# ChainSafe/lumenos

Measured on AMD Instinct MI355X. Metric: prove_eval_seconds_16384x4096, lower is better.
Workload: dtype u64; 1 GPU; Encode+Commit+InnerProduct(r,b)+QueryCols 16384x4096 LogN=14 L=12 K=2 rhoInv=2 queries=309; parallelism=1 GPU: the whole job resident in HBM

## Files before the change

### lumenos_amd/csrc/lm_common.h

```cpp
#pragma once
#include <hip/hip_runtime.h>

#include <algorithm>
#include <cstdarg>
#include <cstdint>
#include <cstdio>
#include <map>
#include <memory>
#include <mutex>
#include <set>
#include <string>
#include <utility>
#include <vector>

#include "../../include/lumenos_hip.h"
#include "lm_arith.h"
#include "lm_dev.h"

#define LM_MAX_LIMBS LUMEN_MAX_LIMBS

struct lm_modmap {
    uint32_t period;
    uint8_t idx[LM_MAX_LIMBS];
};

struct lm_mods {
    mod_t m[LM_MAX_LIMBS];
};

struct lm_prof_entry {
    double total_ms = 0;
    uint64_t launches = 0;
    uint64_t units = 0;
};

struct lm_galois_key {
    lm_dev<u64> d_key;
    lm_dev<uint32_t> d_index;
    lm_dev<uint32_t> d_inv_index;
};

struct lumen_set {
    uint32_t count = 0;
    uint32_t nl = 0;
    uint32_t logw = 0;
    u64 *d = nullptr;
    size_t words = 0;
    bool owner = true;
    lumen_ctx *home = nullptr;
};

struct lm_shared {
    std::recursive_mutex mu;
    lm_dev<tw_t> tw_fwd;
    lm_dev<tw_t> tw_inv;
    std::vector<uint64_t> roots;
    uint32_t fieldN = 0;
    lm_dev<tw_t> scal;
    std::map<uint64_t, lm_galois_key> gkeys;
    std::map<std::string, std::shared_ptr<void>> ext;
};

struct lm_tuning {
    uint32_t ks_batch = 64;
    uint32_t ks_lanes = 0;
    int32_t ks_fused_digits = -1;
    uint32_t ks_close_fused = 1;
    uint32_t debug = 0;
    uint32_t modup_tgroup = 3, moddown_tgroup = 1;
    uint32_t ks_placement = 6;
    uint32_t batch_chunks = 0;
    uint32_t rccl_shared_device = 0;
};

struct lumen_ctx {
    lm_tuning tune;
    std::recursive_mutex mu;
    std::shared_ptr<lm_shared> sh;
    int device = 0;
    hipStream_t stream = nullptr;
    hipStream_t stream2 = nullptr;
    hipEvent_t ev_fork = nullptr, ev_join = nullptr;
    hipStream_t stream_aux = nullptr;
    hipEvent_t ev_aux = nullptr;
    hipEvent_t ev_xdep = nullptr;
    uint32_t aux_digests = 0;
    const u64 *aux_lo = nullptr, *aux_hi = nullptr;
    uint8_t *aux_host = nullptr;
    size_t aux_host_cap = 0;
    void *stage_host = nullptr;
    size_t stage_cap = 0;
    hipEvent_t ev_stage = nullptr;
    void *io_host[2] = {nullptr, nullptr};
    hipEvent_t ev_io[2] = {nullptr, nullptr};
    uint32_t logN = 0, N = 0, L = 0, K = 0;
    uint64_t T = 0;
    uint64_t mod[LM_MAX_LIMBS] = {0};
    uint64_t psi[LM_MAX_LIMBS] = {0};
    lm_mods mods;
    tw_t ninv[LM_MAX_LIMBS];
    std::vector<uint64_t> &roots;
    uint32_t &fieldN;
    std::map<uint64_t, lm_galois_key> &gkeys;
    std::map<std::string, std::shared_ptr<void>> &ext;
    uint64_t mul_counter = 0;
    std::map<std::string, lm_dev<unsigned char>> scratch;
    struct pool_block {
        void *p;
        hipEvent_t ready;
    };
    std::multimap<size_t, pool_block> pool;
    size_t pool_bytes = 0;
    std::set<const void *> lds_attr_done;
    bool prof = false;
    std::map<std::string, lm_prof_entry> prof_tab;
    struct pending_ev {
        std::string name;
        hipEvent_t a, b;
        uint64_t units;
    };
    std::vector<pending_ev> prof_pending;
    std::vector<hipEvent_t> ev_pool;
    hipEvent_t tm0 = nullptr, tm1 = nullptr;
    std::string err;
    explicit lumen_ctx(std::shared_ptr<lm_shared> s)
        : sh(std::move(s)), roots(sh->roots), fieldN(sh->fieldN), gkeys(sh->gkeys), ext(sh->ext) {}
};

static inline size_t lm_ctw(const lumen_ctx *ctx, const lumen_set *s);
#define LM_FULL_WIDTH(ctx, set, what) \
    LM_CHECK(ctx, (set)->logw == 0, "%s: lane-sharded set (1/%u of every limb) where a full-width set is required", what, 1u << (set)->logw)

#define LM_ENTER(ctx)                                             \
    std::lock_guard<std::recursive_mutex> lm_lock_((ctx)->mu);    \
    (void)hipSetDevice((ctx)->device);                            \
    (void)hipGetLastError()
#define LM_SHARED_LOCK(ctx) std::lock_guard<std::recursive_mutex> lm_shlock_((ctx)->sh->mu)

template <class T>
static inline std::shared_ptr<T> lm_ext_get(lumen_ctx *ctx, const std::string &key) {
    LM_SHARED_LOCK(ctx);
    auto it = ctx->ext.find(key);
    return it == ctx->ext.end() ? std::shared_ptr<T>() : std::static_pointer_cast<T>(it->second);
}
static inline void lm_ext_put(lumen_ctx *ctx, const std::string &key, std::shared_ptr<void> v) {
    LM_SHARED_LOCK(ctx);
    ctx->ext[key] = std::move(v);
}

static inline size_t lm_ctw(const lumen_ctx *ctx, const lumen_set *s) { return (size_t)2 * s->nl * (ctx->N >> s->logw); }

void lm_sync_all(lumen_ctx *ctx);
void *lm_stage(lumen_ctx *ctx, size_t bytes);
int lm_h2d_staged(lumen_ctx *ctx, void *dev, const void *host, size_t bytes);
bool lm_host_is_pinned(const void *p);
int lm_h2d(lumen_ctx *ctx, void *dev, const void *host, size_t bytes);
int lm_d2h(lumen_ctx *ctx, void *host, const void *dev, size_t bytes, bool wait);
int lm_h2d_rows(lumen_ctx *ctx, void *dev, size_t dpitch, const void *host, size_t spitch, size_t width, size_t height);

int lm_fail(lumen_ctx *ctx, const char *fmt, ...);
extern thread_local std::string lm_global_err;

#define LM_HIP(ctx, call)                                                                  \
    do {                                                                                   \
        hipError_t e_ = (call);                                                            \
        if (e_ != hipSuccess)                                                              \
            return lm_fail(ctx, "%s failed: %s (%s:%d)", #call, hipGetErrorString(e_),     \
                           __FILE__, __LINE__);                                            \
    } while (0)

#define LM_CHECK(ctx, cond, ...)                    \
    do {                                            \
        if (!(cond)) return lm_fail(ctx, __VA_ARGS__); \
    } while (0)

template <class... P, class... A>
static inline int lm_launch_flat(lumen_ctx *ctx, void (*kernel)(P...), size_t threads, A &&...args) {
    hipLaunchKernelGGL(kernel, dim3((uint32_t)((threads + 255) / 256)), dim3(256), 0, ctx->stream, std::forward<A>(args)...);
    LM_HIP(ctx, hipGetLastError());
    return 0;
}

struct lm_set_guard {
    lumen_ctx *ctx;
    lumen_set *s;
    lm_set_guard(lumen_ctx *c, lumen_set *x) : ctx(c), s(x) {}
    ~lm_set_guard() {
        if (s) lumen_set_destroy(ctx, s);
    }
    lumen_set *release() {
        lumen_set *r = s;
        s = nullptr;
        return r;
    }
    lm_set_guard(lm_set_guard &&o) : ctx(o.ctx), s(o.release()) {}
    lm_set_guard &operator=(const lm_set_guard &) = delete;
};

void lm_set_release_async(lumen_ctx *ctx, lumen_set *set);

void *lm_scratch(lumen_ctx *ctx, const char *name, size_t bytes);
void lm_scratch_adopt(lumen_ctx *ctx, const char *name, void *p, size_t bytes);

struct lm_prof_scope {
    lumen_ctx *ctx;
    const char *name;
    uint64_t units;
    hipEvent_t a = nullptr;
    lm_prof_scope(lumen_ctx *c, const char *n, uint64_t u);
    ~lm_prof_scope();
};
void lm_prof_resolve(lumen_ctx *ctx);

static inline uint64_t h_mulmod(uint64_t a, uint64_t b, uint64_t q) {
    return (uint64_t)(((u128)a * b) % q);
}
static inline uint64_t h_powmod(uint64_t a, uint64_t e, uint64_t q) {
    uint64_t r = 1 % q;
    a %= q;
    while (e) {
        if (e & 1) r = h_mulmod(r, a, q);
        a = h_mulmod(a, a, q);
        e >>= 1;
    }
    return r;
}
static inline uint64_t h_invmod(uint64_t a, uint64_t q) { return h_powmod(a, q - 2, q); }
static inline tw_t h_tw(uint64_t w, uint64_t q) {
    tw_t t;
    t.w = w;
    t.wp = (u64)((((u128)w) << 64) / q);
    return t;
}
static inline uint64_t h_r64_mod(uint64_t q) { return (uint64_t)((((u128)1) << 64) % q); }
static inline uint64_t h_p_mod(const lumen_ctx *ctx, uint64_t q) {
    uint64_t P = 1 % q;
    for (uint32_t a = 0; a < ctx->K; a++) P = h_mulmod(P, ctx->mod[ctx->L + a] % q, q);
    return P;
}
static inline uint32_t h_bitrev(uint32_t x, int bits) {
    uint32_t r = 0;
    for (int i = 0; i < bits; i++) r = (r << 1) | ((x >> i) & 1);
    return r;
}

int lm_launch_ntt(lumen_ctx *ctx, u64 *d, uint32_t npoly, const lm_modmap &map, bool inverse);
struct lm_ninv_t;
int lm_launch_ntt_strided(lumen_ctx *ctx, const u64 *src, size_t src_poly_stride, u64 *dst,
                          size_t dst_poly_stride, uint32_t npoly, const lm_modmap &map, bool inverse,
                          const char *prof_name, const lm_ninv_t *inv_scale = nullptr);
int lm_launch_ntt_subring(lumen_ctx *ctx, uint32_t logn, const tw_t *tw, tw_t ninv_scale, const u64 *src,
                          size_t src_poly_stride, u64 *dst, size_t dst_poly_stride, uint32_t npoly,
                          uint32_t mod_idx, bool inverse, const mod_t *explicit_mod = nullptr);
mod_t lm_make_mod(uint64_t q);
void lm_build_tw(uint64_t q, uint64_t psi, uint32_t logN, std::vector<tw_t> &fwd, std::vector<tw_t> &inv);
int lm_rescale_polys(lumen_ctx *ctx, const u64 *src, uint32_t nl, u64 *dst, uint32_t target,
                     uint32_t npoly, u64 *work, u64 *tbuf);
int lm_rescale_coef_ready(lumen_ctx *ctx);
int lm_rescale_polys_from_coef(lumen_ctx *ctx, const u64 *coef, uint32_t nl, u64 *dst, uint32_t target, uint32_t npoly);
lm_modmap lm_map_q(uint32_t nl);
lm_modmap lm_map_p(const lumen_ctx *ctx);
int lm_encode_dev(lumen_ctx *ctx, const lumen_set *matrix, const u64 *dzero, uint32_t rho_inv, lumen_set **encoded);
int lm_poly_eval_check(lumen_ctx *ctx, const uint64_t *values, uint32_t rows, uint32_t count, uint64_t first_column,
                       uint32_t cols, const char *what);
int lm_poly_eval_enqueue(lumen_ctx *ctx, const uint64_t *values, uint32_t rows, uint32_t count, uint64_t first_column,
                         uint32_t cols, uint64_t z, const char *what);
int lm_poly_eval_finish(lumen_ctx *ctx, uint64_t *partial);
hipEvent_t lm_ev_get(lumen_ctx *ctx);
```

### lumenos_amd/csrc/lm_ctx.hip

```cpp
#include <cstring>
#include <thread>

#include "lm_ntt_dev.h"

thread_local std::string lm_global_err;

int lm_fail(lumen_ctx *ctx, const char *fmt, ...) {
    char buf[1024];
    va_list ap;
    va_start(ap, fmt);
    vsnprintf(buf, sizeof(buf), fmt, ap);
    va_end(ap);
    if (ctx) ctx->err = buf;
    lm_global_err = buf;
    fprintf(stderr, "[lumenos_hip] error: %s\n", buf);
    return 1;
}

void *lm_scratch(lumen_ctx *ctx, const char *name, size_t bytes) {
    auto &e = ctx->scratch[name];
    if (e && e.count() >= bytes) return e.get();
    if (e) lm_sync_all(ctx);
    return e.alloc(ctx, bytes, name) ? nullptr : e.get();
}

void lm_scratch_adopt(lumen_ctx *ctx, const char *name, void *p, size_t bytes) {
    auto &e = ctx->scratch[name];
    if (e.get() == p) (void)e.release();
    if (e) lm_sync_all(ctx);
    e = lm_dev<unsigned char>((unsigned char *)p, bytes);
}

void lm_sync_all(lumen_ctx *ctx) {
    if (ctx->stream) hipStreamSynchronize(ctx->stream);
    if (ctx->stream2) hipStreamSynchronize(ctx->stream2);
    if (ctx->stream_aux) hipStreamSynchronize(ctx->stream_aux);
}

void *lm_stage(lumen_ctx *ctx, size_t bytes) {
    if (ctx->ev_stage) hipEventSynchronize(ctx->ev_stage);
    if (ctx->stage_cap < bytes) {
        if (ctx->stage_host) hipHostFree(ctx->stage_host);
        ctx->stage_host = nullptr, ctx->stage_cap = 0;
        if (hipHostMalloc(&ctx->stage_host, bytes, hipHostMallocDefault) != hipSuccess) {
            lm_fail(ctx, "hipHostMalloc(%zu) for host staging failed", bytes);
            return nullptr;
        }
        ctx->stage_cap = bytes;
    }
    return ctx->stage_host;
}

int lm_h2d_staged(lumen_ctx *ctx, void *dev, const void *host, size_t bytes) {
    void *h = lm_stage(ctx, bytes);
    if (!h) return 1;
    memcpy(h, host, bytes);
    LM_HIP(ctx, hipMemcpyAsync(dev, h, bytes, hipMemcpyHostToDevice, ctx->stream));
    LM_HIP(ctx, hipEventRecord(ctx->ev_stage, ctx->stream));
    return 0;
}

hipEvent_t lm_ev_get(lumen_ctx *ctx) {
    if (!ctx->ev_pool.empty()) {
        hipEvent_t e = ctx->ev_pool.back();
        ctx->ev_pool.pop_back();
        return e;
    }
    hipEvent_t e = nullptr;
    hipEventCreate(&e);
    return e;
}

lm_prof_scope::lm_prof_scope(lumen_ctx *c, const char *n, uint64_t u) : ctx(c), name(n), units(u) {
    if (!ctx->prof) return;
    a = lm_ev_get(ctx);
    hipEventRecord(a, ctx->stream);
}
lm_prof_scope::~lm_prof_scope() {
    if (!ctx->prof || !a) return;
    hipEvent_t b = lm_ev_get(ctx);
    hipEventRecord(b, ctx->stream);
    ctx->prof_pending.push_back({name, a, b, units});
}

void lm_prof_resolve(lumen_ctx *ctx) {
    if (ctx->prof_pending.empty()) return;
    for (auto &p : ctx->prof_pending) {
        float ms = 0;
        if (hipEventSynchronize(p.b) == hipSuccess && hipEventElapsedTime(&ms, p.a, p.b) == hipSuccess) {
            auto &e = ctx->prof_tab[p.name];
            e.total_ms += ms;
            e.launches += 1;
            e.units += p.units;
        } else {
            (void)hipGetLastError();
        }
        ctx->ev_pool.push_back(p.a);
        ctx->ev_pool.push_back(p.b);
    }
    ctx->prof_pending.clear();
}

lm_modmap lm_map_q(uint32_t nl) {
    lm_modmap m;
    m.period = nl;
    for (uint32_t i = 0; i < LM_MAX_LIMBS; i++) m.idx[i] = (uint8_t)(i < nl ? i : 0);
    return m;
}

lm_modmap lm_map_p(const lumen_ctx *ctx) {
    lm_modmap m;
    m.period = ctx->K;
    for (uint32_t i = 0; i < LM_MAX_LIMBS; i++) m.idx[i] = (uint8_t)(ctx->L + (i < ctx->K ? i : 0));
    return m;
}

mod_t lm_make_mod(uint64_t q) {
    mod_t m;
    m.q = q;
    m.qinv64 = (u64)((((u128)1) << 64) / q);
    u64 inv = 1;
    for (int it = 0; it < 6; it++) inv *= 2 - (u64)q * inv;
    m.qneg = (u64)0 - inv;
    u64 r = h_r64_mod(q);
    m.r2 = h_mulmod(r, r, q);
    return m;
}

void lm_build_tw(uint64_t q, uint64_t psi, uint32_t logN, std::vector<tw_t> &fwd, std::vector<tw_t> &inv) {
    uint32_t N = 1u << logN;
    fwd.resize(N);
    inv.resize(N);
    uint64_t psi_inv = h_invmod(psi, q), cf = 1, cb = 1;
    for (uint32_t j = 0; j < N; j++) {
        uint32_t r = h_bitrev(j, (int)logN);
        fwd[r] = h_tw(cf, q);
        inv[r] = h_tw(cb, q);
        cf = h_mulmod(cf, psi, q);
        cb = h_mulmod(cb, psi_inv, q);
    }
}

static void pool_drain(lumen_ctx *ctx) {
    for (auto &kv : ctx->pool) {
        hipFree(kv.second.p);
        if (kv.second.ready) ctx->ev_pool.push_back(kv.second.ready);
    }
    ctx->pool.clear();
    ctx->pool_bytes = 0;
}

static int ctx_private_init(lumen_ctx *ctx) {
    LM_HIP(ctx, hipSetDevice(ctx->device));
    LM_HIP(ctx, hipStreamCreate(&ctx->stream));
    LM_HIP(ctx, hipStreamCreate(&ctx->stream2));
    LM_HIP(ctx, hipEventCreateWithFlags(&ctx->ev_fork, hipEventDisableTiming));
    LM_HIP(ctx, hipEventCreateWithFlags(&ctx->ev_join, hipEventDisableTiming));
    LM_HIP(ctx, hipStreamCreate(&ctx->stream_aux));
    LM_HIP(ctx, hipEventCreateWithFlags(&ctx->ev_aux, hipEventDisableTiming));
    LM_HIP(ctx, hipEventCreateWithFlags(&ctx->ev_stage, hipEventDisableTiming));
    LM_HIP(ctx, hipEventCreateWithFlags(&ctx->ev_xdep, hipEventDisableTiming));
    LM_HIP(ctx, hipEventCreate(&ctx->tm0));
    LM_HIP(ctx, hipEventCreate(&ctx->tm1));
    return 0;
}

static int tuning_set(lm_tuning &t, const char *name, long v) {
    const std::string n(name ? name : "");
    auto in = [&](long lo, long hi) { return v >= lo && v <= hi; };
    if (n == "LUMEN_KS_BATCH") {
        if (!in(1, 4096)) return 2;
        t.ks_batch = (uint32_t)v;
    } else if (n == "LUMEN_KS_LANES") {
        if (!in(0, 2)) return 2;
        t.ks_lanes = (uint32_t)v;
    } else if (n == "LUMEN_KS_FUSED_DIGITS") {
        if (v > LM_MAX_LIMBS) return 2;
        t.ks_fused_digits = v >= 0 ? (int32_t)v : -1;
    } else if (n == "LUMEN_KS_CLOSE_FUSED") {
        if (!in(0, 1)) return 2;
        t.ks_close_fused = (uint32_t)v;
    } else if (n == "LUMEN_DEBUG") {
        t.debug = v != 0;
    } else if (n == "LUMEN_MODUP_TGROUP") {
        if (!in(1, 31)) return 2;
        t.modup_tgroup = (uint32_t)v;
    } else if (n == "LUMEN_MODDOWN_TGROUP") {
        if (!in(1, 31)) return 2;
        t.moddown_tgroup = (uint32_t)v;
    } else if (n == "LUMEN_KS_PLACEMENT") {
        if (!in(0, 32)) return 2;
        t.ks_placement = (uint32_t)v;
    } else if (n == "LUMEN_BATCH_CHUNKS") {
        if (!in(0, 4096)) return 2;
        t.batch_chunks = (uint32_t)v;
    } else {
        return 1;
    }
    return 0;
}
static void tuning_from_env(lm_tuning &t) {
    for (const char *n : {"LUMEN_KS_BATCH", "LUMEN_KS_LANES", "LUMEN_KS_FUSED_DIGITS", "LUMEN_KS_CLOSE_FUSED", "LUMEN_DEBUG",
                          "LUMEN_MODUP_TGROUP", "LUMEN_MODDOWN_TGROUP", "LUMEN_KS_PLACEMENT", "LUMEN_BATCH_CHUNKS"}) {
        const char *e = getenv(n);
        if (e && *e && tuning_set(t, n, atol(e)))
            fprintf(stderr, "[lumenos_hip] %s=%s is out of range: ignored\n", n, e);
    }
}

extern "C" int lumen_ctx_set_tuning(lumen_ctx *ctx, const char *name, long value) {
    LM_CHECK(nullptr, ctx && name, "lumen_ctx_set_tuning: NULL argument");
    LM_ENTER(ctx);
    const int rc = tuning_set(ctx->tune, name, value);
    LM_CHECK(ctx, rc != 1, "unknown tuning switch %s", name);
    LM_CHECK(ctx, rc == 0, "tuning switch %s: value %ld is out of range (nothing changed)", name, value);
    return 0;
}

extern "C" int lumen_test_allow_shared_device_rccl(lumen_ctx *ctx, int on) {
    LM_CHECK(nullptr, ctx, "lumen_test_allow_shared_device_rccl: NULL ctx");
    LM_ENTER(ctx);
    ctx->tune.rccl_shared_device = on != 0;
    return 0;
}

extern "C" int lumen_ctx_wait(lumen_ctx *ctx, lumen_ctx *other) {
    LM_CHECK(nullptr, ctx && other, "lumen_ctx_wait: NULL argument");
    if (ctx == other) return 0;
    hipEvent_t ev;
    {
        LM_ENTER(other);
        LM_HIP(other, hipEventRecord(other->ev_xdep, other->stream));
        ev = other->ev_xdep;
    }
    LM_ENTER(ctx);
    LM_CHECK(ctx, ctx->device == other->device, "lumen_ctx_wait: contexts on devices %d and %d", ctx->device, other->device);
    LM_HIP(ctx, hipStreamWaitEvent(ctx->stream, ev, 0));
    return 0;
}

extern "C" int lumen_ctx_create(const lumen_params_desc *desc, lumen_ctx **out) {
    if (!desc || !out) return lm_fail(nullptr, "lumen_ctx_create: NULL argument");
    *out = nullptr;
    LM_CHECK(nullptr, desc->abi_version == LUMEN_ABI_VERSION, "ABI version mismatch: got %u want %u",
             desc->abi_version, LUMEN_ABI_VERSION);
    LM_CHECK(nullptr, lm_logn_supported(desc->log_n),
             "log_n %u unsupported: kernels are instantiated for N = 2^8 and 2^10..2^14", desc->log_n);
    LM_CHECK(nullptr, desc->num_q >= 1 && desc->num_q + desc->num_p <= LM_MAX_LIMBS,
             "bad limb counts L=%u K=%u", desc->num_q, desc->num_p);
    int ndev = 0;
    if (hipGetDeviceCount(&ndev) != hipSuccess || ndev == 0)
        return lm_fail(nullptr, "no HIP device visible: the lumenos HIP path has no CPU fallback");
    LM_CHECK(nullptr, desc->device >= 0 && desc->device < ndev, "device %d out of range (have %d)",
             desc->device, ndev);
    std::unique_ptr<lumen_ctx, void (*)(lumen_ctx *)> guard(new lumen_ctx(std::make_shared<lm_shared>()),
                                                            lumen_ctx_destroy);
    lumen_ctx *ctx = guard.get();
    tuning_from_env(ctx->tune);
    ctx->device = desc->device;
    ctx->logN = desc->log_n;
    ctx->N = 1u << desc->log_n;
    ctx->L = desc->num_q;
    ctx->K = desc->num_p;
    ctx->T = desc->plaintext_modulus;
    uint32_t LK = ctx->L + ctx->K, N = ctx->N;
    uint64_t two_n = 2ull * N;
    for (uint32_t i = 0; i < LK; i++) {
        uint64_t q = desc->moduli[i], psi = desc->psi[i];
        static_assert(3 * 0 + 8 >= 8, "the modulus bound (3 log_n + 8) q < 2^64 must imply 8 q < 2^64");
        const uint64_t qmax = UINT64_MAX / (3ull * desc->log_n + 8);
        if (q < (1ull << 20) || q > qmax || (q & (two_n - 1)) != 1)
            return lm_fail(nullptr, "modulus %u (%llu) must be == 1 mod 2N and below %llu", i,
                           (unsigned long long)q, (unsigned long long)qmax);
        if (h_powmod(psi, N, q) != q - 1)
            return lm_fail(nullptr, "psi[%u] is not a primitive 2N-th root of unity", i);
        ctx->mod[i] = q;
        ctx->psi[i] = psi;
        ctx->mods.m[i] = lm_make_mod(q);
        ctx->ninv[i] = h_tw(h_invmod(N % q, q), q);
    }
    for (uint32_t i = LK; i < LM_MAX_LIMBS; i++) ctx->mods.m[i] = ctx->mods.m[0];
    if (int rc = ctx_private_init(ctx)) return rc;
    std::vector<tw_t> f, b, fwd, inv;
    for (uint32_t i = 0; i < LK; i++) {
        lm_build_tw(ctx->mod[i], ctx->psi[i], ctx->logN, f, b);
        fwd.insert(fwd.end(), f.begin(), f.end());
        inv.insert(inv.end(), b.begin(), b.end());
    }
    if (ctx->sh->tw_fwd.upload(ctx, fwd, "the forward twiddles") || ctx->sh->tw_inv.upload(ctx, inv, "the inverse twiddles")) return 1;
    *out = guard.release();
    return 0;
}

extern "C" int lumen_ctx_clone(lumen_ctx *src, lumen_ctx **out) {
    if (!src || !out) return lm_fail(nullptr, "lumen_ctx_clone: NULL argument");
    *out = nullptr;
    LM_ENTER(src);
    std::unique_ptr<lumen_ctx, void (*)(lumen_ctx *)> guard(new lumen_ctx(src->sh), lumen_ctx_destroy);
    lumen_ctx *ctx = guard.get();
    ctx->tune = src->tune;
    ctx->device = src->device;
    ctx->logN = src->logN, ctx->N = src->N, ctx->L = src->L, ctx->K = src->K, ctx->T = src->T;
    memcpy(ctx->mod, src->mod, sizeof(ctx->mod));
    memcpy(ctx->psi, src->psi, sizeof(ctx->psi));
    ctx->mods = src->mods;
    memcpy(ctx->ninv, src->ninv, sizeof(ctx->ninv));
    if (int rc = ctx_private_init(ctx)) {
        src->err = ctx->err;
        return rc;
    }
    *out = guard.release();
    return 0;
}

extern "C" void lumen_ctx_destroy(lumen_ctx *ctx) {
    if (!ctx) return;
    {
        LM_ENTER(ctx);
        lm_sync_all(ctx);
        ctx->scratch.clear();
        pool_drain(ctx);
        lm_prof_resolve(ctx);
        for (hipEvent_t e : ctx->ev_pool) hipEventDestroy(e);
        if (ctx->tm0) hipEventDestroy(ctx->tm0);
        if (ctx->tm1) hipEventDestroy(ctx->tm1);
        if (ctx->aux_host) hipHostFree(ctx->aux_host);
        if (ctx->stage_host) hipHostFree(ctx->stage_host);
        for (int i = 0; i < 2; i++) {
            if (ctx->io_host[i]) hipHostFree(ctx->io_host[i]);
            if (ctx->ev_io[i]) hipEventDestroy(ctx->ev_io[i]);
        }
        if (ctx->ev_stage) hipEventDestroy(ctx->ev_stage);
        if (ctx->ev_xdep) hipEventDestroy(ctx->ev_xdep);
        if (ctx->ev_aux) hipEventDestroy(ctx->ev_aux);
        if (ctx->stream_aux) hipStreamDestroy(ctx->stream_aux);
        if (ctx->ev_fork) hipEventDestroy(ctx->ev_fork);
        if (ctx->ev_join) hipEventDestroy(ctx->ev_join);
        if (ctx->stream2) hipStreamDestroy(ctx->stream2);
        if (ctx->stream) hipStreamDestroy(ctx->stream);
        ctx->sh.reset();
    }
    delete ctx;
}

extern "C" int lumen_ctx_trim(lumen_ctx *ctx) {
    LM_CHECK(nullptr, ctx, "lumen_ctx_trim: NULL ctx");
    LM_ENTER(ctx);
    LM_CHECK(ctx, !ctx->aux_digests, "lumen_ctx_trim: a lumen_leaf_digests_begin job is in flight");
    lm_sync_all(ctx);
    for (auto it = ctx->scratch.begin(); it != ctx->scratch.end();) {
        if (it->first == "digests_async" || it->first == "group_digests") {
            ++it;
            continue;
        }
        it = ctx->scratch.erase(it);
    }
    pool_drain(ctx);
    return 0;
}

extern "C" int lumen_ctx_scratch_info(lumen_ctx *ctx, const char *name, void **ptr, size_t *bytes) {
    LM_CHECK(nullptr, ctx && name && ptr, "lumen_ctx_scratch_info: NULL argument");
    LM_ENTER(ctx);
    auto it = ctx->scratch.find(name);
    *ptr = it == ctx->scratch.end() ? nullptr : it->second.get();
    if (bytes) *bytes = it == ctx->scratch.end() ? 0 : it->second.count();
    return 0;
}

extern "C" const char *lumen_last_error(const lumen_ctx *ctx) {
    return ctx ? ctx->err.c_str() : lm_global_err.c_str();
}

extern "C" int lumen_sync(lumen_ctx *ctx) {
    LM_CHECK(nullptr, ctx, "lumen_sync: NULL ctx");
    LM_ENTER(ctx);
    LM_HIP(ctx, hipStreamSynchronize(ctx->stream));
    return 0;
}

extern "C" uint64_t lumen_mul_counter(const lumen_ctx *ctx) { return ctx ? ctx->mul_counter : 0; }

extern "C" int lumen_set_create(lumen_ctx *ctx, uint32_t count, uint32_t num_limbs, lumen_set **out) {
    return lumen_set_create_lanes(ctx, count, num_limbs, 0, out);
}

extern "C" int lumen_set_create_lanes(lumen_ctx *ctx, uint32_t count, uint32_t num_limbs, uint32_t log_world,
                                      lumen_set **out) {
    LM_CHECK(nullptr, ctx && out, "lumen_set_create: NULL argument");
    LM_ENTER(ctx);
    LM_CHECK(ctx, num_limbs >= 1 && num_limbs <= ctx->L, "num_limbs %u out of range [1,%u]", num_limbs, ctx->L);
    LM_CHECK(ctx, log_world <= 6 && (ctx->N >> log_world) >= 64, "a lane shard of 1/%u of N = %u is narrower than 64 coefficients",
             1u << log_world, ctx->N);
    lumen_set *s = new lumen_set();
    s->count = count;
    s->nl = num_limbs;
    s->logw = log_world;
    s->words = (size_t)count * 2 * num_limbs * (ctx->N >> log_world);
    s->home = ctx;
    if (s->words) {
        const size_t bytes = s->words * sizeof(u64);
        auto it = ctx->pool.find(bytes);
        if (it != ctx->pool.end()) {
            s->d = (u64 *)it->second.p;
            if (hipEvent_t ready = it->second.ready) {
                (void)hipStreamWaitEvent(ctx->stream, ready, 0);
                (void)hipStreamWaitEvent(ctx->stream2, ready, 0);
                (void)hipStreamWaitEvent(ctx->stream_aux, ready, 0);
                ctx->ev_pool.push_back(ready);
            }
            ctx->pool.erase(it);
            ctx->pool_bytes -= bytes;
        } else {
            hipError_t e = hipMalloc((void **)&s->d, bytes);
            if (e != hipSuccess && !ctx->pool.empty()) {
                (void)hipGetLastError();
                lm_sync_all(ctx);
                pool_drain(ctx);
                e = hipMalloc((void **)&s->d, bytes);
            }
            if (e != hipSuccess) {
                (void)hipGetLastError();
                delete s;
                return lm_fail(ctx, "hipMalloc(%zu bytes) for a %u x %u-limb set failed: %s", bytes, count,
                               num_limbs, hipGetErrorString(e));
            }
        }
    }
    *out = s;
    return 0;
}

extern "C" void lumen_set_destroy(lumen_ctx *ctx, lumen_set *set) {
    if (!set) return;
    if (ctx) {
        LM_ENTER(ctx);
        hipStreamSynchronize(ctx->stream);
        hipStreamSynchronize(ctx->stream2);
        if (ctx->aux_digests && set->d && set->d < ctx->aux_hi && set->d + set->words > ctx->aux_lo)
            hipStreamSynchronize(ctx->stream_aux);
        if (set->owner && set->d) {
            const size_t bytes = set->words * sizeof(u64);
            if (ctx == set->home && ctx->pool_bytes + bytes <= ((size_t)96 << 30)) {
                ctx->pool.emplace(bytes, lumen_ctx::pool_block{set->d, nullptr});
                ctx->pool_bytes += bytes;
            } else {
                hipFree(set->d);
            }
        }
    } else if (set->owner && set->d) {
        hipFree(set->d);
    }
    delete set;
}

void lm_set_release_async(lumen_ctx *ctx, lumen_set *set) {
    if (!set) return;
    LM_ENTER(ctx);
    const size_t bytes = set->words * sizeof(u64);
    const bool hashing = ctx->aux_digests && set->d && set->d < ctx->aux_hi && set->d + set->words > ctx->aux_lo;
    if (!set->owner || !set->d || ctx != set->home || hashing || ctx->pool_bytes + bytes > ((size_t)96 << 30)) {
        lumen_set_destroy(ctx, set);
        return;
    }
    hipEvent_t ready = lm_ev_get(ctx);
    bool ok = ready && hipEventRecord(ctx->ev_join, ctx->stream2) == hipSuccess &&
              hipStreamWaitEvent(ctx->stream, ctx->ev_join, 0) == hipSuccess && hipEventRecord(ready, ctx->stream) == hipSuccess;
    if (!ok) {
        (void)hipGetLastError();
        if (ready) ctx->ev_pool.push_back(ready);
        lumen_set_destroy(ctx, set);
        return;
    }
    ctx->pool.emplace(bytes, lumen_ctx::pool_block{set->d, ready});
    ctx->pool_bytes += bytes;
    delete set;
}

extern "C" int lumen_set_slice(lumen_ctx *ctx, const lumen_set *set, uint32_t first, uint32_t n,
                               lumen_set **view) {
    LM_CHECK(nullptr, ctx && set && view, "lumen_set_slice: NULL argument");
    LM_ENTER(ctx);
    LM_CHECK(ctx, (uint64_t)first + n <= set->count, "slice [%u,%u) exceeds set of %u", first, first + n, set->count);
    lumen_set *v = new lumen_set();
    const size_t ctw = lm_ctw(ctx, set);
    v->count = n;
    v->nl = set->nl;
    v->logw = set->logw;
    v->d = set->d + (size_t)first * ctw;
    v->words = (size_t)n * ctw;
    v->owner = false;
    *view = v;
    return 0;
}

extern "C" uint32_t lumen_set_count(const lumen_set *set) { return set ? set->count : 0; }
extern "C" uint32_t lumen_set_limbs(const lumen_set *set) { return set ? set->nl : 0; }
extern "C" uint32_t lumen_set_log_world(const lumen_set *set) { return set ? set->logw : 0; }
extern "C" void *lumen_set_device_ptr(const lumen_set *set) { return set ? set->d : nullptr; }

extern "C" void *lumen_host_alloc(size_t bytes) {
    void *p = nullptr;
    if (hipHostMalloc(&p, bytes ? bytes : 1, hipHostMallocDefault) != hipSuccess) {
        (void)hipGetLastError();
        lm_fail(nullptr, "hipHostMalloc(%zu) failed", bytes);
// ... 249 lines not shown
```

### lumenos_amd/csrc/lm_ntt.hip

```cpp
#include "lm_ntt_dev.h"

template <int LOGN, bool INV>
constexpr lm_geom k_limb_ntt_geom = INV ? lm_geom_lds(LOGN) : lm_geom_fwd(LOGN);
template <int LOGN, bool INV>
__global__ LM_GEOM_BOUNDS((k_limb_ntt_geom<LOGN, INV>)) void k_limb_ntt(const u64 *src, size_t src_poly_stride, u64 *dst,
                                                   size_t dst_poly_stride, uint32_t npoly, lm_modmap map,
                                                   lm_mods mods, lm_ninv_t ninv,
                                                   const tw_t *__restrict__ tw_all) {
    extern __shared__ __attribute__((aligned(16))) u64 sm[];
    constexpr uint32_t N = 1u << LOGN;
    const uint32_t tid = threadIdx.x;
    const uint32_t limb = blockIdx.x / npoly, poly = blockIdx.x % npoly;
    const uint32_t mi = map.idx[limb];
    const lm_qc c = lm_make_qc(mods.m[mi]);
    const u64 *p = src + (size_t)poly * src_poly_stride + (size_t)limb * N;
    u64 *o = dst + (size_t)poly * dst_poly_stride + (size_t)limb * N;
    const tw_t *tw = tw_all + (size_t)mi * N;
    if (INV) {
        const tw_t ni = ninv.t[mi];
        auto st = [&](uint32_t i, u64 v) { o[i] = lm_shoup_cs(v, ni, c.q, c.nq); };
        auto ld = [&](uint32_t i0, u64 *v, int count) { lm_load_run(p, i0, v, count); };
        lm_ntt_inverse<LOGN>(sm, tw, c, tid, ld, st);
    } else {
        auto ld = [&](uint32_t i) { return p[i]; };
        auto st = [&](uint32_t i0, const u64 *v, int count) {
            u64 r[8];
#pragma unroll
            for (int k = 0; k < 8; k++)
                if (k < count) r[k] = lm_reduce_s(v[k], c.q, c.nq, c.qinv64);
            lm_store_run(o, i0, r, count);
        };
        if constexpr (LOGN == 14)
            lm_ntt_forward_w14(sm, tw, c, tid, ld, st);
        else
            lm_ntt_forward<LOGN>(sm, tw, c, tid, ld, st);
    }
}

static int launch_limb_ntt(lumen_ctx *ctx, uint32_t logn, bool inverse, uint32_t grid, const u64 *src,
                           size_t src_poly_stride, u64 *dst, size_t dst_poly_stride, uint32_t npoly,
                           const lm_modmap &map, const lm_mods &mods, const lm_ninv_t &ninv, const tw_t *tw) {
    return lm_for_logn(ctx, logn, [&](auto n) {
        if (inverse)
            return lm_launch(ctx, k_limb_ntt<n, true>, k_limb_ntt_geom<n, true>, grid, src, src_poly_stride, dst,
                             dst_poly_stride, npoly, map, mods, ninv, tw);
        return lm_launch(ctx, k_limb_ntt<n, false>, k_limb_ntt_geom<n, false>, grid, src, src_poly_stride, dst,
                         dst_poly_stride, npoly, map, mods, ninv, tw);
    });
}

int lm_launch_ntt_subring(lumen_ctx *ctx, uint32_t logn, const tw_t *tw, tw_t ninv_scale, const u64 *src,
                          size_t src_poly_stride, u64 *dst, size_t dst_poly_stride, uint32_t npoly,
                          uint32_t mod_idx, bool inverse, const mod_t *explicit_mod) {
    if (!npoly) return 0;
    lm_modmap map = lm_map_q(1);
    map.idx[0] = 0;
    lm_mods mods = ctx->mods;
    mods.m[0] = explicit_mod ? *explicit_mod : ctx->mods.m[mod_idx];
    lm_ninv_t ninv = lm_ninv_of(ctx);
    ninv.t[0] = ninv_scale;
    return launch_limb_ntt(ctx, logn, inverse, npoly, src, src_poly_stride, dst, dst_poly_stride, npoly, map, mods, ninv, tw);
}

int lm_launch_ntt_strided(lumen_ctx *ctx, const u64 *src, size_t src_poly_stride, u64 *dst,
                          size_t dst_poly_stride, uint32_t npoly, const lm_modmap &map, bool inverse,
                          const char *prof_name, const lm_ninv_t *inv_scale) {
    if (!npoly || !map.period) return 0;
    const lm_ninv_t ninv = inv_scale ? *inv_scale : lm_ninv_of(ctx);
    const uint64_t nblocks64 = (uint64_t)npoly * map.period;
    LM_CHECK(ctx, nblocks64 < (1ull << 31), "NTT grid too large: %llu", (unsigned long long)nblocks64);
    lm_prof_scope ps(ctx, prof_name ? prof_name : (inverse ? "limb_intt" : "limb_ntt"), nblocks64);
    return launch_limb_ntt(ctx, ctx->logN, inverse, (uint32_t)nblocks64, src, src_poly_stride, dst, dst_poly_stride, npoly,
                           map, ctx->mods, ninv, inverse ? ctx->sh->tw_inv.get() : ctx->sh->tw_fwd.get());
}

int lm_launch_ntt(lumen_ctx *ctx, u64 *d, uint32_t npoly, const lm_modmap &map, bool inverse) {
    const size_t stride = (size_t)map.period * ctx->N;
    return lm_launch_ntt_strided(ctx, d, stride, d, stride, npoly, map, inverse, nullptr, nullptr);
}

extern "C" int lumen_set_ntt(lumen_ctx *ctx, lumen_set *set, int inverse) {
    LM_CHECK(nullptr, ctx && set, "lumen_set_ntt: NULL argument");
    LM_ENTER(ctx);
    LM_FULL_WIDTH(ctx, set, "lumen_set_ntt");
    return lm_launch_ntt(ctx, set->d, set->count * 2, lm_map_q(set->nl), inverse != 0);
}
```

### lumenos_amd/csrc/lm_ntt_dev.h

```cpp
#pragma once
#include <cstring>
#include <type_traits>
#include <utility>

#include "lm_common.h"

#define LM_PAD(i) ((i) + ((i) >> 3))
template <int LOG_STRIDE>
__device__ __forceinline__ uint32_t lm_pad_at(uint32_t base, uint32_t pbase, int k) {
    if constexpr (LOG_STRIDE >= 3)
        return pbase + (uint32_t)k * ((1u << LOG_STRIDE) + (1u << (LOG_STRIDE - 3)));
    else
        return LM_PAD(base + ((uint32_t)k << LOG_STRIDE));
}
#define LM_MAX_PASSES 8

struct lm_ninv_t {
    tw_t t[LM_MAX_LIMBS];
};

__host__ __device__ constexpr int lm_ilog2(int x) { return x <= 1 ? 0 : 1 + lm_ilog2(x >> 1); }
__host__ __device__ constexpr size_t lm_lds_for(uint32_t n) { return (size_t)(n + (n >> 3) + 2) * sizeof(u64); }
struct lm_geom {
    int threads;
// ... 428 lines not shown
template <class Loader, class Storer>
__device__ __forceinline__ void lm_fwd14_xpass(u64 *sm, const tw_t *tw, const lm_qc &c, uint32_t tid, Loader &ld,
                                               Storer &st) {
    constexpr int LOGN = 14;
    static_assert(lm_npasses(LOGN) == 4 && lm_pass_r(LOGN, 0) == 4 && lm_pass_r(LOGN, 1) == 4 &&
                      lm_pass_r(LOGN, 2) == 3 && lm_pass_r(LOGN, 3) == 3,
                  "written for the pass plan 4 | 4 3 3");
    using D4 = lm_deal<LOGN, 4>;
    using D3 = lm_deal<LOGN, 3>;
    static_assert(D4::reps == 1 && D3::reps == 2, "one item in pass 1, two in passes 2 and 3");
    lm_fwd_first<LOGN, 4, true>(sm, tw, c, tid, ld);
    lm_twset<4, true> T1;
    T1.load(tw, 4, D4::local(tid, 0) >> (LOGN - 8));
    __syncthreads();
    lm_twset<3, false> A, B;
    A.load(tw, 8, D3::local(tid, 0) >> (LOGN - 11));
    B.load(tw, 8, D3::local(tid, 1) >> (LOGN - 11));
    lm_fwd_mid_item<LOGN, 4, 4, true>(sm, T1, c, D4::local(tid, 0));
    lm_wave_sync();
    lm_fwd_mid_item<LOGN, 3, 8, false>(sm, A, c, D3::local(tid, 0));
    A.load(tw, 11, D3::local(tid, 0));
    lm_fwd_mid_item<LOGN, 3, 8, false>(sm, B, c, D3::local(tid, 1));
    B.load(tw, 11, D3::local(tid, 1));
    lm_wave_sync();
#pragma unroll
    for (uint32_t m = 0; m < 2; m++) {
        const uint32_t base = D3::local(tid, m) << 3;
        u64 e[8];
#pragma unroll
        for (int k = 0; k < 8; k++) e[k] = sm[LM_PAD(base + k)];
        lm_fwd_stages<3, false>(e, m ? B : A, c);
        st(base, e, 8);
    }
}

template <int LOGN, bool XPASS = true, class Loader, class Storer, class After = lm_no_after>
__device__ __forceinline__ void lm_ntt_forward(u64 *sm, const tw_t *tw, const lm_qc &c, uint32_t tid, Loader &ld,
                                               Storer &st, After after = After()) {
    static_assert(lm_npasses(LOGN) >= 2, "a transform needs a loading and a storing pass");
    if constexpr (LOGN == 14 && XPASS && LM_TW_XPASS && !lm_has_pre<Storer>::value)
        lm_fwd14_xpass(sm, tw, c, tid, ld, st);
    else
        lm_fwd_rec<LOGN, 0, 0>(sm, tw, c, tid, ld, st);
    after(0u, 1u << LOGN);
}

#define LM_W14_THREADS 512
#ifndef LM_W14_SCHED_FENCE
#define LM_W14_SCHED_FENCE 1
#endif
#if LM_W14_SCHED_FENCE
#define LM_W14_FENCE() __builtin_amdgcn_sched_barrier(0)
#else
#define LM_W14_FENCE() ((void)0)
#endif
#ifndef LM_W14_PF3
#define LM_W14_PF3 0
#endif
#ifndef LM_W14_PF4
#define LM_W14_PF4 0
#endif
struct lm_w14_plan {
    static constexpr int R1 = 5, R2 = 3, R3 = 3, R4 = 3;
};
static_assert(lm_w14_plan::R1 + lm_w14_plan::R2 + lm_w14_plan::R3 + lm_w14_plan::R4 == 14, "the four passes cover the 14 stages once");
static_assert((1 << lm_w14_plan::R1) == 32 && (1 << lm_w14_plan::R2) * 4 == 32 && (1 << lm_w14_plan::R3) * 4 == 32 &&
                  (1 << lm_w14_plan::R4) * 4 == 32,
              "pass 1 is one item of 32 coefficients per lane, passes 2-4 four items of 8");
static_assert(LM_W14_THREADS * 32 == 1 << 14 && LM_W14_THREADS / 64 == 8, "8 waves x 64 lanes x 32 coefficients");
__device__ __forceinline__ uint32_t lm_w14_pos(uint32_t i) { return LM_PAD(((i >> 11) << 10) | (i & 1023u)); }
__device__ __forceinline__ uint32_t lm_w14_at(uint32_t pbase, uint32_t k) { return pbase + k + (k >> 3); }

template <int R>
__device__ __forceinline__ void lm_fwd_stages_first(u64 *e, const tw_t *tw, const lm_qc &c) {
#pragma unroll
    for (int st = 0; st < R; st++) {
        const int span = (1 << R) >> st, half = span >> 1, CH = half < 8 ? half : 8;
#pragma unroll
        for (int g = 0; g < (1 << st); g++) {
            const tw_t W = lm_tw_load<true>(tw, (1u << st) + g);
#pragma unroll
            for (int k0 = 0; k0 < half; k0 += CH) {
                u64 sum[CH];
#pragma unroll
                for (int k = 0; k < CH; k++)
                    sum[k] = lm_shoup3<true>(e[g * span + k0 + k + half], W.w, W.wp, c.nq, e[g * span + k0 + k]);
#pragma unroll
                for (int k = 0; k < CH; k++) {
                    u64 &x = e[g * span + k0 + k];
                    e[g * span + k0 + k + half] = lm_bfly_diff(x, c.q3, sum[k]);
                    x = sum[k];
                }
            }
        }
    }
}

template <class Loader, class Storer, class After = lm_no_after>
__device__ __forceinline__ void lm_ntt_forward_w14(u64 *sm, const tw_t *tw, const lm_qc &c, uint32_t tid, Loader &ld,
                                                   Storer &st, After after = After()) {
    const uint32_t w = tid >> 6, l = tid & 63;
    u64 e[32];
#pragma unroll
    for (int r = 0; r < 32; r++) e[r] = ld(((uint32_t)r << 9) | tid);
    lm_fwd_stages_first<5>(e, tw, c);
    const uint32_t p1 = LM_PAD(tid), p2 = LM_PAD((w << 10) | l);
    lm_twset<3, true> T2[2];
    T2[0].load(tw, 5, (w << 2) | 0);
    u64 e0[16];
#pragma unroll
    for (int h = 0; h < 2; h++) {
#pragma unroll
        for (int r = 0; r < 32; r++)
            if (((r >> 1) & 1) == h) sm[lm_w14_at(p1, (uint32_t)((r >> 2) << 10 | (r & 1) << 9))] = e[r];
        __syncthreads();
#pragma unroll
        for (int r = 0; r < 16; r++) (h ? e[16 + r] : e0[r]) = sm[lm_w14_at(p2, (uint32_t)r << 6)];
        if (h == 0) __syncthreads();
    }
#pragma unroll
    for (int r = 0; r < 16; r++) e[r] = e0[r];
#pragma unroll
    for (int gq = 0; gq < 4; gq++) {
        if (gq + 1 < 4) T2[(gq + 1) & 1].load(tw, 5, (w << 2) | (uint32_t)(gq + 1));
        lm_fwd_stages<3, true>(e + 8 * gq, T2[gq & 1], c);
    }
    const uint32_t p3 = LM_PAD((w << 10) | ((l >> 3) << 6) | (l & 7));
    lm_twset<3, false> T3[2];
    T3[0].load(tw, 8, (w << 5) | (l >> 3));
#pragma unroll
    for (int h = 0; h < 2; h++) {
        lm_wave_sync();
#pragma unroll
        for (int r = 16 * h; r < 16 * h + 16; r++) sm[lm_w14_at(p2, (uint32_t)(r & 15) << 6)] = e[r];
        lm_wave_sync();
#pragma unroll
        for (int r = 16 * h; r < 16 * h + 16; r++)
            e[r] = sm[lm_w14_at(p3, (uint32_t)(((r >> 3) & 1) << 9 | (r & 7) << 3))];
    }
#pragma unroll
    for (int m = 0; m < 4; m++) {
        LM_W14_FENCE();
        if (LM_W14_PF3 && m + 1 < 4) T3[(m + 1) & 1].load(tw, 8, (w << 5) | ((uint32_t)(m + 1) << 3) | (l >> 3));
        if (!LM_W14_PF3 && m) T3[0].load(tw, 8, (w << 5) | ((uint32_t)m << 3) | (l >> 3));
        lm_fwd_stages<3, false>(e + 8 * m, T3[LM_W14_PF3 ? (m & 1) : 0], c);
    }
    const uint32_t p4 = LM_PAD((w << 10) | (l << 3));
    lm_twset<3, false> T4[2];
    T4[0].load(tw, 11, (w << 8) | l);
#pragma unroll
    for (int h = 0; h < 2; h++) {
        lm_wave_sync();
#pragma unroll
        for (int r = 16 * h; r < 16 * h + 16; r++)
            sm[lm_w14_at(p3, (uint32_t)(((r >> 3) & 1) << 9 | (r & 7) << 3))] = e[r];
        lm_wave_sync();
#pragma unroll
        for (int r = 16 * h; r < 16 * h + 16; r++)
            e[r] = sm[lm_w14_at(p4, (uint32_t)(((r >> 3) & 1) << 9 | (r & 7)))];
    }
    constexpr bool TWPF = LM_W14_PF4 && !lm_has_pre<Storer>::value;
    lm_wave_sync();
#pragma unroll
    for (int m = 0; m < 4; m++) {
        LM_W14_FENCE();
        const uint32_t i0 = (w << 11) | ((uint32_t)m << 9) | (l << 3);
        if constexpr (lm_has_pre<Storer>::value) st.pre(i0);
        if (TWPF && m + 1 < 4) T4[(m + 1) & 1].load(tw, 11, (w << 8) | ((uint32_t)(m + 1) << 6) | l);
        if (!TWPF && m) T4[0].load(tw, 11, (w << 8) | ((uint32_t)m << 6) | l);
        lm_fwd_stages<3, false>(e + 8 * m, T4[TWPF ? (m & 1) : 0], c);
        st(i0, e + 8 * m, 8);
        if (m & 1) {
            lm_wave_sync();
            after((uint32_t)(m >> 1) << 10, 1024u);
            lm_wave_sync();
        }
    }
}
struct lm_w14_runs {
    u64 *sm;
    __device__ __forceinline__ void operator()(uint32_t i0, const u64 *v, int count) const {
        const uint32_t pb = lm_w14_pos(i0);
#pragma unroll
        for (int k = 0; k < 8; k++)
            if (k < count) sm[pb + k] = v[k];
    }
};
template <class F>
__device__ __forceinline__ void lm_w14_linear_out(const u64 *sm, uint32_t tid, uint32_t i0, F f) {
    const uint32_t w = tid >> 6, lane = tid & 63;
    const uint32_t pb = LM_PAD((w << 10) | (2 * lane));
#pragma unroll
    for (uint32_t k = 0; k < 8; k++) {
        const uint32_t j = (w << 11) | i0 | (2 * lane + 128 * k);
        f(j, sm[lm_w14_at(pb, 128 * k)], sm[lm_w14_at(pb, 128 * k) + 1]);
    }
}

__host__ __device__ constexpr lm_geom lm_geom_fwd(int logN) {
    return logN == 14 ? lm_geom{LM_W14_THREADS, 4, lm_lds_for(1u << 13)} : lm_geom_lds(logN);
}

template <int LOGN, int R, class Loader>
__device__ __forceinline__ void lm_inv_first(u64 *s, const tw_t *tw, const lm_qc &c, uint32_t tid, Loader &ld) {
    using D = lm_deal<LOGN, R>;
    if (!D::valid(tid)) return;
#pragma unroll 1
    for (uint32_t m = 0; m < D::reps; m++) {
        const uint32_t w = D::local(tid, m);
        const uint32_t base = w << R;
        u64 e[1 << R];
        lm_inv_twset<R, false, true> T;
        T.load(tw, LOGN, 0, w);
        ld(base, e, 1 << R);
        lm_inv_stages<R, false, false, true>(e, T, c);
#pragma unroll
        for (int k = 0; k < (1 << R); k++) s[LM_PAD(base + k)] = e[k];
    }
}

#ifndef LM_INV_TW_PREFETCH
#define LM_INV_TW_PREFETCH 1
#endif
template <int LOGN, int R, int LT>
__device__ __forceinline__ void lm_inv_mid(u64 *s, const tw_t *tw, const lm_qc &c, uint32_t tid) {
    using D = lm_deal<LOGN, R>;
    if (!D::valid(tid)) return;
    constexpr bool UW = LT >= 6;
    lm_inv_twset<R, UW, false> T[2];
    T[0].load(tw, LOGN, LT, D::local(tid, 0) >> LT);
#pragma unroll
    for (uint32_t m = 0; m < D::reps; m++) {
        const uint32_t w = D::local(tid, m);
        const uint32_t blk = w >> LT, off = w & ((1u << LT) - 1);
        const uint32_t base = (blk << (LT + R)) + off;
        u64 e[1 << R];
        const uint32_t pb = LM_PAD(base);
#pragma unroll
        for (int k = 0; k < (1 << R); k++) e[k] = s[lm_pad_at<LT>(base, pb, k)];
        if (LM_INV_TW_PREFETCH && m + 1 < D::reps) T[(m + 1) & 1].load(tw, LOGN, LT, D::local(tid, m + 1) >> LT);
        if (!LM_INV_TW_PREFETCH && m) T[0].load(tw, LOGN, LT, blk);
        lm_inv_stages<R, UW, false, false>(e, T[LM_INV_TW_PREFETCH ? (m & 1) : 0], c);
#pragma unroll
        for (int k = 0; k < (1 << R); k++) s[lm_pad_at<LT>(base, pb, k)] = e[k];
    }
}

template <class S, class = void>
struct lm_has_slot : std::false_type {};
template <class S>
struct lm_has_slot<S, std::void_t<decltype(std::declval<S &>()(0u, (u64)0, 0))>> : std::true_type {};

template <int LOGN, int R, class Storer>
__device__ __forceinline__ void lm_inv_last(const u64 *s, const tw_t *tw, const lm_qc &c, uint32_t tid, Storer &st) {
    constexpr uint32_t log_t0 = LOGN - R, items = 1u << log_t0, NT = lm_nthreads(LOGN);
    constexpr uint32_t reps = items / NT ? items / NT : 1;
    lm_inv_twset<R, true, false> T;
    T.load(tw, LOGN, log_t0, 0);
#pragma unroll 1
    for (uint32_t m = 0; m < reps; m++) {
        const uint32_t w = tid + m * NT;
        if (items < NT && w >= items) break;
        u64 e[1 << R];
#pragma unroll
        for (int k = 0; k < (1 << R); k++) e[k] = s[lm_pad_at<log_t0>(w, LM_PAD(w), k)];
        if constexpr (lm_has_pre<Storer>::value) st.pre(w);
        lm_inv_stages<R, true, true, false>(e, T, c);
#pragma unroll
        for (int k = 0; k < (1 << R); k++) {
            if constexpr (lm_has_slot<Storer>::value)
                st(w + ((uint32_t)k << log_t0), e[k], k);
            else
                st(w + ((uint32_t)k << log_t0), e[k]);
        }
    }
}

template <int LOGN, int P, int LT, class Loader, class Storer>
__device__ __forceinline__ void lm_inv_rec(u64 *sm, const tw_t *tw, const lm_qc &c, uint32_t tid, Loader &ld,
                                           Storer &st) {
    constexpr int NP = lm_npasses(LOGN), R = lm_pass_r(LOGN, NP - 1 - P);
    constexpr bool cross = lm_cross_r(LOGN) > 0;
    if constexpr (P == 0)
        lm_inv_first<LOGN, R>(sm, tw, c, tid, ld);
    else if constexpr (P == NP - 1)
        lm_inv_last<LOGN, R>(sm, tw, c, tid, st);
    else
        lm_inv_mid<LOGN, R, LT>(sm, tw, c, tid);
    if constexpr (P + 1 < NP) {
        if constexpr (P + 2 == NP && cross)
            __syncthreads();
        else
            lm_wave_sync();
        lm_inv_rec<LOGN, P + 1, LT + R>(sm, tw, c, tid, ld, st);
    }
}
template <int LOGN, class Loader, class Storer>
__device__ __forceinline__ void lm_ntt_inverse(u64 *sm, const tw_t *tw, const lm_qc &c, uint32_t tid, Loader &ld,
                                               Storer &st) {
    static_assert(lm_npasses(LOGN) >= 2, "a transform needs a loading and a storing pass");
    lm_inv_rec<LOGN, 0, 0>(sm, tw, c, tid, ld, st);
}

__device__ __forceinline__ void lm_load_run(const u64 *p, uint32_t i0, u64 *v, int count) {
    if (count == 2) {
        const ulonglong2 a = *reinterpret_cast<const ulonglong2 *>(p + i0);
        v[0] = a.x, v[1] = a.y;
    } else {
#pragma unroll
        for (int k = 0; k < 8; k += 2) {
            if (k < count) {
                const ulonglong2 a = *reinterpret_cast<const ulonglong2 *>(p + i0 + k);
                v[k] = a.x, v[k + 1] = a.y;
            }
        }
    }
}
struct lm_lds_runs {
    u64 *sm;
    __device__ __forceinline__ void operator()(uint32_t i0, const u64 *v, int count) const {
#pragma unroll
        for (int k = 0; k < 8; k++)
            if (k < count) sm[LM_PAD(i0 + k)] = v[k];
    }
};
template <int LOGN, class F>
__device__ __forceinline__ void lm_linear_out(const u64 *sm, uint32_t tid, F f) {
    constexpr uint32_t NW = lm_nthreads(LOGN) / 64, BLK = (1u << LOGN) / NW, IT = BLK / 128 ? BLK / 128 : 1;
    const uint32_t wave = tid >> 6, lane = tid & 63;
    lm_wave_sync();
#pragma unroll
    for (uint32_t k = 0; k < IT; k++) {
        const uint32_t j = wave * BLK + 2 * lane + k * 128;
        if (BLK >= 128 || 2 * lane < BLK) f(j, sm[LM_PAD(j)], sm[LM_PAD(j + 1)]);
    }
}

__device__ __forceinline__ void lm_store_run(u64 *p, uint32_t i0, const u64 *v, int count) {
#pragma unroll
    for (int k = 0; k < 8; k += 2) {
        if (k < count) {
            ulonglong2 a;
            a.x = v[k], a.y = v[k + 1];
            *reinterpret_cast<ulonglong2 *>(p + i0 + k) = a;
        }
    }
}
```

Before: 1.705 s.

## Add register-resident wide inverse NTT kernel for logN 14

New measurement: 1.716 s. About the same (+0.7%).

```diff
diff --git a/lumenos_amd/csrc/lm_common.h b/lumenos_amd/csrc/lm_common.h
--- a/lumenos_amd/csrc/lm_common.h
+++ b/lumenos_amd/csrc/lm_common.h
@@ -66,6 +66,7 @@
     uint32_t ks_lanes = 0;
     int32_t ks_fused_digits = -1;
     uint32_t ks_close_fused = 1;
+    int32_t intt_w14 = -1;
     uint32_t debug = 0;
     uint32_t modup_tgroup = 3, moddown_tgroup = 1;
     uint32_t ks_placement = 6;
diff --git a/lumenos_amd/csrc/lm_ctx.hip b/lumenos_amd/csrc/lm_ctx.hip
--- a/lumenos_amd/csrc/lm_ctx.hip
+++ b/lumenos_amd/csrc/lm_ctx.hip
@@ -180,6 +180,9 @@
     } else if (n == "LUMEN_KS_CLOSE_FUSED") {
         if (!in(0, 1)) return 2;
         t.ks_close_fused = (uint32_t)v;
+    } else if (n == "LUMEN_INTT_W14") {
+        if (v > 1) return 2;
+        t.intt_w14 = v >= 0 ? (int32_t)v : -1;
     } else if (n == "LUMEN_DEBUG") {
         t.debug = v != 0;
     } else if (n == "LUMEN_MODUP_TGROUP") {
@@ -200,7 +203,7 @@
     return 0;
 }
 static void tuning_from_env(lm_tuning &t) {
-    for (const char *n : {"LUMEN_KS_BATCH", "LUMEN_KS_LANES", "LUMEN_KS_FUSED_DIGITS", "LUMEN_KS_CLOSE_FUSED", "LUMEN_DEBUG",
+    for (const char *n : {"LUMEN_KS_BATCH", "LUMEN_KS_LANES", "LUMEN_KS_FUSED_DIGITS", "LUMEN_KS_CLOSE_FUSED", "LUMEN_INTT_W14", "LUMEN_DEBUG",
                           "LUMEN_MODUP_TGROUP", "LUMEN_MODDOWN_TGROUP", "LUMEN_KS_PLACEMENT", "LUMEN_BATCH_CHUNKS"}) {
         const char *e = getenv(n);
         if (e && *e && tuning_set(t, n, atol(e)))
diff --git a/lumenos_amd/csrc/lm_ntt.hip b/lumenos_amd/csrc/lm_ntt.hip
--- a/lumenos_amd/csrc/lm_ntt.hip
+++ b/lumenos_amd/csrc/lm_ntt.hip
@@ -37,9 +37,39 @@
     }
 }
 
+__global__ LM_GEOM_BOUNDS(lm_geom_inv(14)) void k_limb_intt_w14(const u64 *src, size_t src_poly_stride, u64 *dst,
+                                                                size_t dst_poly_stride, uint32_t npoly, lm_modmap map,
+                                                                lm_mods mods, lm_ninv_t ninv,
+                                                                const tw_t *__restrict__ tw_all) {
+    extern __shared__ __attribute__((aligned(16))) u64 sm[];
+    constexpr uint32_t N = 1u << 14;
+    const uint32_t limb = blockIdx.x / npoly, poly = blockIdx.x % npoly;
+    const uint32_t mi = map.idx[limb];
+    const lm_qc c = lm_make_qc(mods.m[mi]);
+    const u64 *p = src + (size_t)poly * src_poly_stride + (size_t)limb * N;
+    u64 *o = dst + (size_t)poly * dst_poly_stride + (size_t)limb * N;
+    const tw_t ni = ninv.t[mi];
+    auto st = [&](uint32_t i, u64 v) { o[i] = lm_shoup_cs(v, ni, c.q, c.nq); };
+    auto ld = [&](uint32_t i0, u64 *v, int count) { lm_load_run(p, i0, v, count); };
+    lm_ntt_inverse_w14(sm, tw_all + (size_t)mi * N, c, threadIdx.x, ld, st);
+}
+static bool use_intt_w14(lumen_ctx *ctx, uint32_t logn, uint32_t grid) {
+    if (logn != 14 || ctx->tune.intt_w14 == 0) return false;
+    if (ctx->tune.intt_w14 > 0) return true;
+    static const uint32_t cus = [&] {
+        int n = 0;
+        if (hipDeviceGetAttribute(&n, hipDeviceAttributeMultiprocessorCount, ctx->device) != hipSuccess || n < 1) n = 256;
+        return (uint32_t)n;
+    }();
+    return grid > cus;
+}
+
 static int launch_limb_ntt(lumen_ctx *ctx, uint32_t logn, bool inverse, uint32_t grid, const u64 *src,
                            size_t src_poly_stride, u64 *dst, size_t dst_poly_stride, uint32_t npoly,
                            const lm_modmap &map, const lm_mods &mods, const lm_ninv_t &ninv, const tw_t *tw) {
+    if (inverse && use_intt_w14(ctx, logn, grid))
+        return lm_launch(ctx, k_limb_intt_w14, lm_geom_inv(14), grid, src, src_poly_stride, dst, dst_poly_stride, npoly, map, mods,
+                         ninv, tw);
     return lm_for_logn(ctx, logn, [&](auto n) {
         if (inverse)
             return lm_launch(ctx, k_limb_ntt<n, true>, k_limb_ntt_geom<n, true>, grid, src, src_poly_stride, dst,
diff --git a/lumenos_amd/csrc/lm_ntt_dev.h b/lumenos_amd/csrc/lm_ntt_dev.h
--- a/lumenos_amd/csrc/lm_ntt_dev.h
+++ b/lumenos_amd/csrc/lm_ntt_dev.h
@@ -754,6 +754,124 @@
     lm_inv_rec<LOGN, 0, 0>(sm, tw, c, tid, ld, st);
 }
 
+__device__ __forceinline__ void lm_inv_w14_item(u64 *e, const tw_t *tw, uint32_t log_t0, uint32_t blk, const lm_qc &c) {
+    lm_inv_twset<3, false, false> T;
+    T.load(tw, 14, log_t0, blk);
+    lm_inv_stages<3, false, false, false>(e, T, c);
+}
+template <class Loader, class Storer>
+__device__ __forceinline__ void lm_ntt_inverse_w14(u64 *sm, const tw_t *tw, const lm_qc &c, uint32_t tid, Loader &ld,
+                                                   Storer &st) {
+    const uint32_t w = tid >> 6, l = tid & 63;
+    u64 e[32];
+#pragma unroll
+    for (int m = 0; m < 4; m++) ld((w << 11) | ((uint32_t)m << 9) | (l << 3), e + 8 * m, 8);
+#pragma unroll
+    for (int m = 0; m < 4; m++) {
+        LM_W14_FENCE();
+        lm_inv_w14_item(e + 8 * m, tw, 0, (w << 8) | ((uint32_t)m << 6) | l, c);
+    }
+    LM_W14_FENCE();
+    const uint32_t p4 = LM_PAD((w << 10) | (l << 3));
+    const uint32_t p3 = LM_PAD((w << 10) | ((l >> 3) << 6) | (l & 7));
+#pragma unroll
+    for (int h = 0; h < 2; h++) {
+        lm_wave_sync();
+#pragma unroll
+        for (int r = 16 * h; r < 16 * h + 16; r++)
+            sm[lm_w14_at(p4, (uint32_t)(((r >> 3) & 1) << 9 | (r & 7)))] = e[r];
+        lm_wave_sync();
+#pragma unroll
+        for (int r = 16 * h; r < 16 * h + 16; r++)
+            e[r] = sm[lm_w14_at(p3, (uint32_t)(((r >> 3) & 1) << 9 | (r & 7) << 3))];
+    }
+#pragma unroll
+    for (int m = 0; m < 4; m++) {
+        LM_W14_FENCE();
+        lm_inv_w14_item(e + 8 * m, tw, 3, (w << 5) | ((uint32_t)m << 3) | (l >> 3), c);
+    }
+    LM_W14_FENCE();
+    const uint32_t p2 = LM_PAD((w << 10) | l);
+#pragma unroll
+    for (int h = 0; h < 2; h++) {
+        lm_wave_sync();
+#pragma unroll
+        for (int r = 16 * h; r < 16 * h + 16; r++)
+            sm[lm_w14_at(p3, (uint32_t)(((r >> 3) & 1) << 9 | (r & 7) << 3))] = e[r];
+        lm_wave_sync();
+#pragma unroll
+        for (int r = 16 * h; r < 16 * h + 16; r++) e[r] = sm[lm_w14_at(p2, (uint32_t)(r & 15) << 6)];
+    }
+#pragma unroll
+    for (int gq = 0; gq < 4; gq++) {
+        LM_W14_FENCE();
+        lm_inv_twset<3, true, false> T2;
+        T2.load(tw, 14, 6, (w << 2) | (uint32_t)gq);
+        lm_inv_stages<3, true, false, false>(e + 8 * gq, T2, c);
+    }
+    LM_W14_FENCE();
+    const uint32_t p1 = LM_PAD(tid);
+    u64 f[32];
+#pragma unroll
+    for (int h = 0; h < 2; h++) {
+        lm_wave_sync();
+#pragma unroll
+        for (int r = 16 * h; r < 16 * h + 16; r++) sm[lm_w14_at(p2, (uint32_t)(r & 15) << 6)] = e[r];
+        __syncthreads();
+#pragma unroll
+        for (int r = 0; r < 32; r++)
+            if (((r >> 1) & 1) == h) f[r] = sm[lm_w14_at(p1, (uint32_t)((r >> 2) << 10 | (r & 1) << 9))];
+        if (h == 0) __syncthreads();
+    }
+    uint32_t ts = tid;
+    asm volatile("" : "+v"(ts));
+#pragma unroll
+    for (int g0 = 0; g0 < 16; g0 += 8) {
+        u64 dif[8];
+#pragma unroll
+        for (int g = 0; g < 8; g++) {
+            u64 &x = f[2 * (g0 + g)], &y = f[2 * (g0 + g) + 1];
+            dif[g] = x + c.q3 - y;
+            x = lm_csub(x + y, c.q3);
+        }
+#pragma unroll
+        for (int g = 0; g < 8; g++) {
+            const tw_t W = lm_tw_load<true>(tw, 16u + (uint32_t)(g0 + g));
+            f[2 * (g0 + g) + 1] = lm_shoup3<true>(dif[g], W.w, W.wp, c.nq);
+        }
+    }
+#pragma unroll
+    for (int s4 = 0; s4 < 4; s4++) {
+        const int half = 2 << s4, span = half << 1, CH = half < 8 ? half : 8;
+        const u64 C = c.q3 << s4;
+#pragma unroll
+        for (int g = 0; g < 32 / span; g++) {
+            const tw_t W = lm_tw_load<true>(tw, (8u >> s4) + (uint32_t)g);
+#pragma unroll
+            for (int k0 = 0; k0 < half; k0 += CH) {
+                u64 dif[CH];
+#pragma unroll
+                for (int k = 0; k < CH; k++) {
+                    u64 &x = f[g * span + k0 + k], &y = f[g * span + k0 + k + half];
+                    dif[k] = x + C - y;
+                    x = x + y;
+                }
+#pragma unroll
+                for (int k = 0; k < CH; k++) f[g * span + k0 + k + half] = lm_shoup3<true>(dif[k], W.w, W.wp, c.nq);
+            }
+        }
+    }
+#pragma unroll
+    for (int r = 0; r < 32; r++) {
+        if constexpr (lm_has_slot<Storer>::value)
+            st(((uint32_t)r << 9) | ts, f[r], r);
+        else
+            st(((uint32_t)r << 9) | ts, f[r]);
+        if ((r & 3) == 3) LM_W14_FENCE();
+    }
+}
+__host__ __device__ constexpr lm_geom lm_geom_inv(int logN) { return lm_geom_fwd(logN); }
+
 __device__ __forceinline__ void lm_load_run(const u64 *p, uint32_t i0, u64 *v, int count) {
     if (count == 2) {
         const ulonglong2 a = *reinterpret_cast<const ulonglong2 *>(p + i0);
```
